# broadinstitute/Tangram

Measured on NVIDIA H100. Metric: map_cells_to_space iterations/sec, higher is better.
Workload: dtype bf16 operands / f32 accumulate+state

## Files before the change

### tangram_b200/csrc/adam_rows.cuh

```cuda
#pragma once
#include "common.cuh"
#include "gemm_tc.cuh"

namespace tgb {

struct AdamRowsArgs {
  float* M; __nv_bfloat16* m; float* v;
  const __nv_bfloat16* dq;
  __nv_bfloat16* Pt;
  const RowConst* rowc;
  float* zsum; float* pxsum; float* l1sum; float* l2sum;
  int ld, V, row0, row1;
  float lam_r, lam_l1, lam_l2;
  AdamScalars a;
};

__device__ __forceinline__ void ldg256f(const float* src, float (&x)[8]) {
  asm volatile("ld.global.cs.v4.f32 {%0,%1,%2,%3}, [%8];\n\t"
               "ld.global.cs.v4.f32 {%4,%5,%6,%7}, [%8+16];"
               : "=f"(x[0]), "=f"(x[1]), "=f"(x[2]), "=f"(x[3]), "=f"(x[4]), "=f"(x[5]), "=f"(x[6]), "=f"(x[7]) : "l"(src));
}
__device__ __forceinline__ void stg256f(float* dst, const float (&x)[8]) {
  asm volatile("st.global.cs.v4.f32 [%0], {%1,%2,%3,%4};\n\t"
               "st.global.cs.v4.f32 [%0+16], {%5,%6,%7,%8};"
// ... 13 lines not shown
  for (int e = 0; e < 4; ++e) {
    const __nv_bfloat162 b = *reinterpret_cast<const __nv_bfloat162*>(&w[e]);
    f[2 * e] = __low2float(b); f[2 * e + 1] = __high2float(b);
  }
}
__device__ __forceinline__ uint4 pack_bf8(const float (&f)[8]) {
  uint4 o;
  __nv_bfloat162 b;
  b = __floats2bfloat162_rn(f[0], f[1]); o.x = *reinterpret_cast<uint32_t*>(&b);
  b = __floats2bfloat162_rn(f[2], f[3]); o.y = *reinterpret_cast<uint32_t*>(&b);
  b = __floats2bfloat162_rn(f[4], f[5]); o.z = *reinterpret_cast<uint32_t*>(&b);
  b = __floats2bfloat162_rn(f[6], f[7]); o.w = *reinterpret_cast<uint32_t*>(&b);
  return o;
}

#ifndef TGB_ADAM_MAXNREG
#define TGB_ADAM_MAXNREG 96
#endif
template <bool PLAIN>
__global__ void __maxnreg__(TGB_ADAM_MAXNREG)
k_adam_rows(const AdamRowsArgs p) {
  const int lane = threadIdx.x & 31;
  const int row = p.row0 + blockIdx.x * 8 + (threadIdx.x >> 5);
  if (row >= p.row1) return;
  const RowConst rc = p.rowc[row];
  const float lse_l2e = rc.lse * 1.4426950408889634f;
  const size_t base = (size_t)row * p.ld;
  float* Mr = p.M + base; __nv_bfloat16* mr = p.m + base; float* vr = p.v + base;
  const __nv_bfloat16* dr = p.dq + base;
  __nv_bfloat16* pr = p.Pt + base;

  const float k_nstep = -p.a.step_size;

  float zs = 0.f, pxs = 0.f, l1s = 0.f, l2s = 0.f;

  auto load = [&](int c, AdamRowsLoad& L) {
    ldg256f(Mr + c, L.x); L.mq = ldg128_stream(mr + c); ldg256f(vr + c, L.v);
    L.d = ldg128_stream(dr + c);
  };
// ... 70 lines not shown
  if (c < p.ld) {
    AdamRowsLoad A;
    load(c, A);
    process(c, A);
  }
  zs = warp_sum(zs);
  if (p.pxsum) pxs = warp_sum(pxs);
  if (p.l1sum) { l1s = warp_sum(l1s); l2s = warp_sum(l2s); }
  if (lane == 0) {
    p.zsum[row] = zs;
    if (p.pxsum) p.pxsum[row] = pxs;
    if (p.l1sum) { p.l1sum[row] = l1s; p.l2sum[row] = l2s; }
  }
}

struct AdamRowsExactArgs {
  float* M; float* m; float* v;
  const float* dp;
  const RowStat* stats; const float* rdot;
  int ld, V, row0, row1;
  float lam_r, lam_l1, lam_l2;
  AdamScalars a;
};

__global__ void __launch_bounds__(256)
k_adam_rows_exact(const AdamRowsExactArgs p) {
  const int lane = threadIdx.x & 31;
  const int row = p.row0 + blockIdx.x * 8 + (threadIdx.x >> 5);
  if (row >= p.row1) return;
  const RowStat st = p.stats[row];
// ... 15 lines not shown
        if (p.lam_l2 != 0.f) g += 2.f * p.lam_l2 * x[e];
        x[e] = adam_update(x[e], g, m[e], v[e], p.a);
      }
    }
    stg256f(Mr + c, x); stg256f(mr + c, m); stg256f(vr + c, v);
  }
}

static inline int adam_rows_exact_launch(const AdamRowsExactArgs& a, cudaStream_t s) {
  const int rows = a.row1 - a.row0;
  if (rows <= 0) return 0;
  k_adam_rows_exact<<<(unsigned)ceil_div(rows, 8), 256, 0, s>>>(a);
  return cudaGetLastError() == cudaSuccess ? 0 : -2;
}

static inline int adam_rows_launch(const AdamRowsArgs& a, cudaStream_t s) {
  const int rows = a.row1 - a.row0;
  if (rows <= 0) return 0;
  const unsigned grid = (unsigned)ceil_div(rows, 8);
  const bool plain = a.lam_r == 0.f && a.lam_l1 == 0.f && a.lam_l2 == 0.f;
  if (plain) k_adam_rows<true><<<grid, 256, 0, s>>>(a);
  else k_adam_rows<false><<<grid, 256, 0, s>>>(a);
  return cudaGetLastError() == cudaSuccess ? 0 : -2;
}

}
```

### tangram_b200/csrc/gemm_tc.cuh

```cuda
#pragma once
#include <cuda.h>
#include <cstdio>
#include "common.cuh"
#include "gemm_simt.cuh"

namespace tgb {

constexpr int TC_BM = 128;
constexpr int TC_BK = 64;
constexpr int TC_MMA_K = 16;
constexpr int TC_BN = 256;
constexpr int TC_THREADS = 384;
constexpr int TC_ACC = TC_BN / 2;

__device__ __forceinline__ uint32_t smem_u32(const void* p) { return (uint32_t)__cvta_generic_to_shared(p); }

__device__ __forceinline__ void mbar_init(uint64_t* bar, uint32_t count) {
  asm volatile("mbarrier.init.shared::cta.b64 [%0], %1;" ::"r"(smem_u32(bar)), "r"(count));
}
__device__ __forceinline__ void mbar_expect_tx(uint64_t* bar, uint32_t bytes) {
  asm volatile("mbarrier.arrive.expect_tx.shared::cta.b64 _, [%0], %1;" ::"r"(smem_u32(bar)), "r"(bytes) : "memory");
}
__device__ __forceinline__ void mbar_wait(uint64_t* bar, uint32_t parity) {
  asm volatile(
// ... 486 lines not shown
  const long long kps = ((k_total + s - 1) / s + TC_BK - 1) / TC_BK * TC_BK;
  return (int)((k_total + kps - 1) / kps);
}
static inline int tc_splits_for_chain(long long k_total, int max_chain) {
  long long s = (k_total + max_chain - 1) / max_chain;
  if (s < 1) s = 1;
  const long long kps = ((k_total + s - 1) / s + TC_BK - 1) / TC_BK * TC_BK;
  return (int)((k_total + kps - 1) / kps);
}
static inline int tc_forward_splits(int num_sms, int N, int V, int Ke) {
  return tc_splits(num_sms, (long long)ceil_div(V, TC_BM) * ceil_div(Ke, TC_BN), N, 512);
}
static inline int tc_kps(int k_total, int splits) {
  return (int)(round_up(ceil_div(k_total, splits), TC_BK));
}
static inline unsigned tc_grid(const TcContext& tc, long long total) {
  return (unsigned)(total < tc.num_sms ? total : tc.num_sms);
}

static inline int tc_make_maps(TcContext& tc, TcMaps* maps, const __nv_bfloat16* base, size_t plane_elems, int n_planes,
                               uint64_t cols, uint64_t rows, uint64_t ld, uint32_t bi, uint32_t bo, char* err, size_t n) {
  for (int p = 0; p < 3; ++p) {
    const __nv_bfloat16* ptr = base + (size_t)(p < n_planes ? p : 0) * plane_elems;
    if (tc_make_map(tc, &maps->m[p], ptr, cols, rows, ld, bi, bo, err, n)) return -2;
  }
  return 0;
}

struct TcPlan {
  TcMaps a, b;
  CUtensorMap pt, dq;
  bool ready = false;
};

static inline int tc_forward_plan(TcContext& tc, TcPlan& pl, const __nv_bfloat16* P, size_t p_plane, const __nv_bfloat16* Sx,
                                  size_t s_plane, int planes, int N, int V, int Ke, int ld, char* err, size_t n) {
  if (tc_make_maps(tc, &pl.a, P, p_plane, planes, V, N, ld, 64, 64, err, n)) return -2;
  if (tc_make_maps(tc, &pl.b, Sx, s_plane, planes, Ke, N, Ke, 64, 64, err, n)) return -2;
  pl.ready = true;
  return 0;
}
static inline int tc_forward_launch(TcContext& tc, const TcPlan& pl, int n_pairs, float* out, int N, int V, int Ke, int splits,
                                    cudaStream_t s, char* err, size_t n) {
  auto kern = k_gemm_tc<false, false, tc_stages<TcEpiStore>(), TcEpiStore>;
  if (tc_set_smem(tc, kern, TC_SMEM, err, n)) return -2;
  TcEpiStore epi{out, Ke, (size_t)V * Ke, V, 0};
  const int tm = (int)ceil_div(V, TC_BM), tn = (int)ceil_div(Ke, TC_BN);
  kern<<<tc_grid(tc, (long long)tm * tn * splits), TC_THREADS, TC_SMEM, s>>>(pl.a, pl.b, n_pairs, N, tc_kps(N, splits), tm, tn,
                                                                             splits, 1, kPolicyEvictNormal, kPolicyEvictNormal, 0, 0, epi);
  return tc_check_launch("tc_gemm_fwd", err, n);
}
static inline int tc_forward_launch_rows(TcContext& tc, const TcPlan& pl, float* out, int accumulate, int row0, int row1, int V, int Ke,
                                         cudaStream_t s, char* err, size_t n) {
  auto kern = k_gemm_tc<false, false, tc_stages<TcEpiStore>(), TcEpiStore>;
  if (tc_set_smem(tc, kern, TC_SMEM, err, n)) return -2;
  TcEpiStore epi{out, Ke, (size_t)V * Ke, V, accumulate};
  const int tm = (int)ceil_div(V, TC_BM), tn = (int)ceil_div(Ke, TC_BN);
  kern<<<tc_grid(tc, (long long)tm * tn), TC_THREADS, TC_SMEM, s>>>(pl.a, pl.b, 1, row1, (int)round_up(row1 - row0, TC_BK), tm, tn,
                                                                    1, 1, kPolicyEvictNormal, kPolicyEvictNormal, 0, row0, epi);
  return tc_check_launch("tc_gemm_fwd", err, n);
}
static inline int tc_forward(TcContext& tc, const __nv_bfloat16* P, size_t p_plane, const __nv_bfloat16* Sx, size_t s_plane,
                             int n_pairs, float* out, int N, int V, int Ke, int ld, int splits, cudaStream_t s, char* err,
                             size_t n) {
  TcPlan pl;
  if (tc_forward_plan(tc, pl, P, p_plane, Sx, s_plane, n_pairs > 1 ? 3 : 1, N, V, Ke, ld, err, n)) return -2;
  return tc_forward_launch(tc, pl, n_pairs, out, N, V, Ke, splits, s, err, n);
}

static inline int tc_dpstore_plan(TcContext& tc, TcPlan& pl, const __nv_bfloat16* Sxb, size_t s_plane, const __nv_bfloat16* dYb,
                                  size_t dy_plane, int planes, int N, int V, int Ke, char* err, size_t n) {
  if (tc_make_maps(tc, &pl.a, Sxb, s_plane, planes, Ke, N, Ke, 64, TC_BM, err, n)) return -2;
  if (tc_make_maps(tc, &pl.b, dYb, dy_plane, planes, Ke, V, Ke, 64, TC_BN, err, n)) return -2;
  pl.ready = true;
  return 0;
}
static inline int tc_dpstore_epi_plan(TcContext& tc, TcPlan& pl, const __nv_bfloat16* Pt, const __nv_bfloat16* dq, int N, int ld,
                                      char* err, size_t n) {
  if (tc_make_map(tc, &pl.pt, Pt, ld, N, ld, 64, 64, err, n)) return -2;
  return tc_make_map(tc, &pl.dq, dq, ld, N, ld, 64, 64, err, n);
}
template <class Epi>
static inline int tc_dpstore_launch(TcContext& tc, const TcPlan& pl, int n_pairs, const Epi& epi, int row0, int row1, int V, int Ke,
                                    cudaStream_t s, char* err, size_t n) {
  const int tn = (int)ceil_div(V, TC_BN);
  auto kern = k_gemm_tc<true, true, tc_stages<Epi>(), Epi>;
  constexpr int smem = tc_smem<Epi>();
  if (tc_set_smem(tc, kern, smem, err, n)) return -2;
  const int tm0 = row0 / TC_BM, tm = (int)ceil_div(row1, TC_BM) - tm0;
  kern<<<tc_grid(tc, (long long)tm * tn), TC_THREADS, smem, s>>>(pl.a, pl.b, n_pairs, Ke, Ke, tm, tn, 1, 1,
                                                                 kPolicyEvictNormal, kPolicyEvictLast, tm0, 0, epi);
  return tc_check_launch("tc_gemm_bwd_dp", err, n);
}

}
```

### tangram_b200/csrc/tangram_b200.cu

```cuda
#include "../../include/tangram_b200.h"

#include <algorithm>
#include <cmath>
#include <cstdarg>
#include <cstdio>
#include <cstdlib>
#include <cstring>
#include <mutex>
#include <string>
#include <thread>
#include <vector>

#include "common.cuh"
#include "kernels_elem.cuh"
#include "gemm_simt.cuh"
#include "gemm_tc.cuh"
#include "adam_rows.cuh"
#include "legacy_rng.cuh"
#include "agreement.cuh"
#include "annotate.cuh"
#include "mt19937_jump.h"
#include "nccl_dl.h"

using namespace tgb;
// ... 98 lines not shown
  DevBuf<float> colfin;
  DevBuf<float> hist;
  int64_t hist_len = 0, hist_cap = 0;
  bool have_expr = false, have_density = false, have_ct = false, have_mapping = false;
  bool in_step = false;
  int64_t launches = 0;
  float legacy_stats[8] = {0};
  TcContext tc;
  TcPlan plan_fwd, plan_dp;
  DevBuf<__nv_bfloat16> dq;
  DevBuf<__nv_bfloat16> mb;
  DevBuf<float> rcenter;
  DevBuf<float> dpf;
  bool pipelined = false;
  int nchunks = 1, chunk_row[9] = {0};
  cudaStream_t hi = nullptr, lo = nullptr, sf = nullptr;
  cudaEvent_t ev_fork = nullptr, ev_join_hi = nullptr, ev_join_lo = nullptr, ev_join_sf = nullptr, ev_loss = nullptr;
  cudaEvent_t ev_g[8] = {}, ev_a[8] = {}, ev_f[8] = {};
  bool a_valid = false;
  bool prefetch_next = false;
  bool fwd_ahead = false;
  bool defer_join = false;
  bool serial = false;
  bool recording = false;
  std::vector<LaunchRecord> records;
  void drop_records(size_t from) {
    for (size_t i = from; i < records.size(); ++i) cudaEventDestroy(records[i].ev);
    records.resize(from);
  }
  void* comm = nullptr;
  bool comm_owned = false;
  int comm_rank = 0, comm_world = 1;
  bool y_nccl = false;
  void* y_reg = nullptr;
  void release_exchange_registration() {
    if (!y_nccl) return;
    char e[64];
    if (NcclApi* a = nccl_api(e, sizeof(e))) {
      if (y_reg && comm) a->CommDeregister(comm, y_reg);
      a->MemFree(Y.p);
    }
    Y.p = nullptr; Y.n = 0; y_nccl = false; y_reg = nullptr;
  }
  ~tgb200_mapper() {
    release_exchange_registration();
    if (comm && comm_owned) { char e[64]; if (NcclApi* a = nccl_api(e, sizeof(e))) a->CommDestroy(comm); }
    if (hi) cudaStreamDestroy(hi);
    if (lo) cudaStreamDestroy(lo);
    if (sf) cudaStreamDestroy(sf);
    for (cudaEvent_t e : {ev_fork, ev_join_hi, ev_join_lo, ev_join_sf, ev_loss}) if (e) cudaEventDestroy(e);
    for (int i = 0; i < 8; ++i)
      for (cudaEvent_t e : {ev_g[i], ev_a[i], ev_f[i]}) if (e) cudaEventDestroy(e);
    drop_records(0);
  }
};

static void mark(tgb200_mapper* h, cudaStream_t s, const char* name) {
  h->launches++;
  if (!h->recording) return;
  cudaEvent_t e;
  cudaEventCreate(&e);
  cudaEventRecord(e, s);
  h->records.push_back({name, s == h->hi ? 1 : (s == h->lo ? 2 : (s == h->sf ? 3 : 0)), e});
}
#define LAUNCH_CHECK(name)                                                                  \
  do {                                                                                      \
    cudaError_t e__ = cudaGetLastError();                                                   \
    if (e__ != cudaSuccess) return fail(TGB200_ERR_CUDA, "launch %s: %s", name, cudaGetErrorString(e__)); \
    mark(h, s, name);                                                                       \
  } while (0)

static float* s_act(tgb200_mapper* h) { return h->constrained ? h->Sf.p : h->Sx.p; }

static bool needs_rowaux(const tgb200_config& c) { return c.lambda_l1 != 0.f || c.lambda_l2 != 0.f; }
static bool needs_rowscalars(const tgb200_config& c) {
  return c.lambda_r != 0.f || c.lambda_l1 != 0.f || c.lambda_l2 != 0.f;
}

extern "C" int tgb200_host_pin(void* buf, int64_t bytes, int32_t threads, int32_t device) {
  if (!buf || bytes <= 0) return fail(TGB200_ERR_INVALID, "bad argument");
  CK(cudaSetDevice(device));
  const size_t page = 4096, n = (size_t)bytes;
  const int nt = threads < 1 ? 1 : (threads > 32 ? 32 : threads);
  volatile unsigned char* b = static_cast<volatile unsigned char*>(buf);
  auto touch = [=](size_t lo, size_t hi) { for (size_t o = lo; o < hi; o += page) b[o] = 0; };
// ... 85 lines not shown
  A(h->d.alloc(h->V)); A(h->dsrc.alloc(h->N));
  A(h->stats.alloc(h->N)); A(h->rowaux.alloc((size_t)2 * h->N)); A(h->rdot.alloc(h->N));
  if (h->bf16) {
    int nc = h->N >= 32768 ? 4 : (h->N >= 8192 ? 2 : 1);
    if (const char* e = getenv("TGB200_CHUNKS")) nc = atoi(e);
    if (nc < 1) nc = 1;
    if (nc > 8) nc = 8;
    if (h->constrained) nc = 1;
    while (nc > 1 && h->N / nc < 1024) --nc;
    h->nchunks = nc;
    for (int c = 0; c <= nc; ++c) h->chunk_row[c] = c == nc ? h->N : (int)round_up((int64_t)c * h->N / nc, 256);
  }
  if (h->nchunks > 1) {
    int lo_p = 0, hi_p = 0;
    cudaDeviceGetStreamPriorityRange(&lo_p, &hi_p);
    const int mid_p = hi_p < lo_p ? hi_p + 1 : lo_p;
    bool ok = cudaStreamCreateWithPriority(&h->hi, cudaStreamNonBlocking, hi_p) == cudaSuccess &&
              cudaStreamCreateWithPriority(&h->sf, cudaStreamNonBlocking, mid_p) == cudaSuccess &&
              cudaStreamCreateWithPriority(&h->lo, cudaStreamNonBlocking, lo_p) == cudaSuccess;
    cudaEvent_t* evs[5] = {&h->ev_fork, &h->ev_join_hi, &h->ev_join_lo, &h->ev_join_sf, &h->ev_loss};
    for (auto e : evs) ok = ok && cudaEventCreateWithFlags(e, cudaEventDisableTiming) == cudaSuccess;
    for (int c = 0; c < 8; ++c)
      ok = ok && cudaEventCreateWithFlags(&h->ev_g[c], cudaEventDisableTiming) == cudaSuccess &&
           cudaEventCreateWithFlags(&h->ev_a[c], cudaEventDisableTiming) == cudaSuccess &&
           cudaEventCreateWithFlags(&h->ev_f[c], cudaEventDisableTiming) == cudaSuccess;
    if (!ok) A(fail(TGB200_ERR_CUDA, "stream / event creation failed: %s", cudaGetErrorString(cudaGetLastError())));
    h->pipelined = ok;
  }
  h->tc.num_sms = prop.multiProcessorCount;
  if (h->nchunks > 1) {
    h->fwd_splits = 1;
  } else if (h->tcm) {
    h->fwd_splits = tc_forward_splits(h->tc.num_sms, h->N, h->V, h->Ke);
    if (h->x3) h->fwd_splits = std::max(h->fwd_splits, tc_splits_for_chain(h->N, 2048));
  } else {
    const int tiles = (int)(ceil_div(h->V, 128) * ceil_div(h->Ke, 128));
    h->fwd_splits = std::clamp((int)ceil_div(2 * h->tc.num_sms, tiles), 1, (int)ceil_div(h->N, 512));
  }
  if (h->fwd_splits > 1) A(h->Ypart.alloc((size_t)h->fwd_splits * vk));
  A(h->Y.alloc(vk + kTail));
  if (!h->tcm) A(h->dY.alloc(vk));
  if (h->constrained) {
    A(h->Fl.alloc(h->N)); A(h->mF.alloc(h->N)); A(h->vF.alloc(h->N)); A(h->fsig.alloc(h->N));
    A(h->Sf.alloc((size_t)h->N * h->Ke)); A(h->fscal.alloc(4));
// ... 183 lines not shown

static int zero_moments(tgb200_mapper* h, cudaStream_t s) {
  if (h->bf16) CK(cudaMemsetAsync(h->mb.p, 0, h->mb.n * sizeof(__nv_bfloat16), s));
  else CK(cudaMemsetAsync(h->m.p, 0, h->m.n * sizeof(float), s));
  CK(cudaMemsetAsync(h->v.p, 0, h->v.n * sizeof(float), s));
  return TGB200_OK;
}

static int reset_optimizer(tgb200_mapper* h, cudaStream_t s) {
  CKS(zero_moments(h, s));
  if (h->bf16) CK(cudaMemsetAsync(h->rcenter.p, 0, h->rcenter.n * sizeof(float), s));
  h->step = 0;
  h->hist_len = 0;
  h->in_step = false;
  h->p_state = PState::stale;
  h->fwd_ahead = false;
  return TGB200_OK;
}

extern "C" int tgb200_reset_adam(tgb200_mapper* h, void* stream) {
  if (!h) return fail(TGB200_ERR_INVALID, "null handle");
  if (h->in_step) return fail(TGB200_ERR_STATE, "reset_adam inside a step");
  cudaStream_t s = (cudaStream_t)stream;
  CK(cudaSetDevice(h->cfg.device));
  CKS(zero_moments(h, s));
  if (h->constrained) {
    CK(cudaMemsetAsync(h->mF.p, 0, h->mF.n * sizeof(float), s));
    CK(cudaMemsetAsync(h->vF.p, 0, h->vF.n * sizeof(float), s));
  }
  h->step = 0;
  return TGB200_OK;
// ... 339 lines not shown

static cudaStream_t work_stream(tgb200_mapper* h, cudaStream_t s) { return (h->pipelined && !h->serial) ? h->hi : s; }
static cudaStream_t update_stream(tgb200_mapper* h, cudaStream_t s) { return (h->pipelined && !h->serial) ? h->lo : s; }
static int fork_streams(tgb200_mapper* h, cudaStream_t s) {
  if (!h->pipelined || h->serial || h->defer_join) return TGB200_OK;
  CK(cudaEventRecord(h->ev_fork, s));
  CK(cudaStreamWaitEvent(h->hi, h->ev_fork, 0));
  return TGB200_OK;
}
static int join_streams(tgb200_mapper* h, cudaStream_t s) {
  if (!h->pipelined || h->serial || h->defer_join) return TGB200_OK;
  CK(cudaEventRecord(h->ev_join_hi, h->hi));
  CK(cudaStreamWaitEvent(s, h->ev_join_hi, 0));
  CK(cudaEventRecord(h->ev_join_lo, h->lo));
  CK(cudaStreamWaitEvent(s, h->ev_join_lo, 0));
  CK(cudaEventRecord(h->ev_join_sf, h->sf));
  CK(cudaStreamWaitEvent(s, h->ev_join_sf, 0));
  return TGB200_OK;
}

static int forward_chunk(tgb200_mapper* h, cudaStream_t s, int c, int fresh, const float* lseA, float* lseT) {
  float* rowaux = needs_rowaux(h->cfg) ? h->rowaux.p : nullptr;
  if (!h->plan_fwd.ready)
    CKS(tc_forward_plan(h->tc, h->plan_fwd, h->Pb.p, (size_t)h->N * h->ld, h->Sxs.p, (size_t)h->N * h->Ke, 1, h->N, h->V, h->Ke, h->ld,
                        g_err, sizeof(g_err)));
  const int r0 = h->nchunks > 1 ? h->chunk_row[c] : 0, r1 = h->nchunks > 1 ? h->chunk_row[c + 1] : h->N;
  if (h->a_valid && h->pipelined && !h->serial) CK(cudaStreamWaitEvent(s, h->ev_a[c], 0));
  k_row_norm<<<(unsigned)ceil_div(r1 - r0, 256), 256, 0, s>>>(fresh, h->zsum.p, h->pxsum.p, h->l1sum.p, h->l2sum.p,
                                                             lseA, lseT, h->inv_zt.p, h->stats.p, rowaux, r0, r1);
  LAUNCH_CHECK("row_norm");
  const long long nq = (long long)(r1 - r0) * (h->Ke / 4);
  k_scale_rows_bf16<<<(unsigned)ceil_div(nq, 256), 256, 0, s>>>(s_act(h), h->inv_zt.p, r0, r1, h->Ke, h->Sxs.p);
  LAUNCH_CHECK("scale_rows");
  if (h->nchunks > 1) {
    CKS(tc_forward_launch_rows(h->tc, h->plan_fwd, h->Y.p, c > 0 ? 1 : 0, r0, r1, h->V, h->Ke, s, g_err, sizeof(g_err)));
    mark(h, s, "tc_gemm_fwd");
  }
  return TGB200_OK;
}

static int forward_pass(tgb200_mapper* h, cudaStream_t s, int want_entropy) {
  float* rowaux = needs_rowaux(h->cfg) ? h->rowaux.p : nullptr;
  if (h->bf16) {
    if (h->p_state == PState::stale) {
      CKS(launch_softmax_rows<__nv_bfloat16>(h, s, h->Pb.p, 1, rowaux));
      h->p_state = PState::fresh;
    }
    if (h->fwd_ahead) {
      h->fwd_ahead = false;
      for (int c = 0; c < h->nchunks; ++c) CK(cudaStreamWaitEvent(s, h->ev_f[c], 0));
      if (h->nchunks > 1) return TGB200_OK;
    } else {
      for (int c = 0; c < h->nchunks; ++c) CKS(forward_chunk(h, s, c, h->p_state == PState::fresh ? 1 : 0, h->lseA, h->lseT));
    }
    if (h->nchunks > 1) return TGB200_OK;
  } else if (h->x3) {
    CKS(launch_softmax_rows<float>(h, s, (float*)nullptr, want_entropy, rowaux, Split3{h->Pb.p, (size_t)h->N * h->ld}));
  } else {
    CKS(launch_softmax_rows<float>(h, s, h->Pf.p, want_entropy, rowaux));
  }
  const size_t vk = (size_t)h->V * h->Ke;
  float* out = h->fwd_splits > 1 ? h->Ypart.p : h->Y.p;
  if (h->tcm) {
    if (!h->plan_fwd.ready) {
      const __nv_bfloat16* sB = h->bf16 ? h->Sxs.p : h->Sxb.p;
      CKS(tc_forward_plan(h->tc, h->plan_fwd, h->Pb.p, (size_t)h->N * h->ld, sB, (size_t)h->N * h->Ke, h->x3 ? 3 : 1, h->N, h->V, h->Ke,
                          h->ld, g_err, sizeof(g_err)));
    }
    CKS(tc_forward_launch(h->tc, h->plan_fwd, h->x3 ? 6 : 1, out, h->N, h->V, h->Ke, h->fwd_splits, s, g_err, sizeof(g_err)));
// ... 124 lines not shown

static int filter_update(tgb200_mapper* h, cudaStream_t s, const AdamScalars& a) {
  const AdamScalarsF af{a.one_minus_beta1, a.beta2, a.one_minus_beta2, a.step_size, a.bc2_sqrt, a.eps};
  k_filter_update<<<(unsigned)ceil_div(h->N, 256), 256, 0, s>>>(h->N, h->rdot.p, h->fsig.p, h->fscal.p, h->cfg.lambda_count,
                                                                 h->cfg.lambda_f_reg, af, h->Fl.p, h->mF.p, h->vF.p);
  LAUNCH_CHECK("filter_update");
  return TGB200_OK;
}

static int backward_bf16(tgb200_mapper* h, cudaStream_t s, cudaStream_t su, const AdamScalars& a) {
  if (!h->plan_dp.ready) {
    CKS(tc_dpstore_epi_plan(h->tc, h->plan_dp, h->Pb.p, h->dq.p, h->N, h->ld, g_err, sizeof(g_err)));
    CKS(tc_dpstore_plan(h->tc, h->plan_dp, h->Sxb.p, 0, h->dYb.p, 0, 1, h->N, h->V, h->Ke, g_err, sizeof(g_err)));
  }
  const bool two_streams = su != s;
  const bool prefetch = two_streams && h->prefetch_next && h->nchunks > 1 && !h->constrained;
  for (int c = 0; c < h->nchunks; ++c) {
    const int r0 = h->nchunks > 1 ? h->chunk_row[c] : 0, r1 = h->nchunks > 1 ? h->chunk_row[c + 1] : h->N;
    TcEpiDpStore epi{h->plan_dp.pt, h->plan_dp.dq, h->ld, h->rcenter.p, h->rpart.p, h->N};
    CKS(tc_dpstore_launch(h->tc, h->plan_dp, 1, epi, r0, r1, h->V, h->Ke, s, g_err, sizeof(g_err)));
    mark(h, s, "tc_gemm_bwd_dp");
    if (two_streams) {
      CK(cudaEventRecord(h->ev_g[c], s));
      CK(cudaStreamWaitEvent(su, h->ev_g[c], 0));
    }
    k_rowdot_finalize_staged<<<(unsigned)ceil_div(r1 - r0, 256), 256, 0, su>>>(h->rpart.p, h->r_parts, h->N, r0, r1, h->lseT, h->inv_zt.p,
                                                                               h->stats.p, h->rcenter.p, h->rdot.p, h->rowc.p);
    { cudaStream_t s = su; LAUNCH_CHECK("rowdot_finalize"); }
    if (h->constrained) CKS(filter_update(h, su, a));
    AdamRowsArgs ar{h->M.p, h->mb.p, h->v.p, h->dq.p, h->Pb.p, reinterpret_cast<const RowConst*>(h->rowc.p),
                    h->zsum.p, h->pxsum.p, h->l1sum.p, h->l2sum.p, h->ld, h->V, r0, r1,
                    h->cfg.lambda_r, h->cfg.lambda_l1, h->cfg.lambda_l2, a};
    if (adam_rows_launch(ar, su)) return fail(TGB200_ERR_CUDA, "launch adam_rows: %s", cudaGetErrorString(cudaGetLastError()));
    mark(h, su, "adam_rows");
    if (two_streams) CK(cudaEventRecord(h->ev_a[c], su));
    h->a_valid = two_streams;
    if (prefetch) {
      if (c == 0) CK(cudaStreamWaitEvent(h->sf, h->ev_loss, 0));
      CKS(forward_chunk(h, h->sf, c, 0, h->lseT, h->lseA));
      CK(cudaEventRecord(h->ev_f[c], h->sf));
    }
  }
  h->fwd_ahead = prefetch;
  float* t = h->lseA; h->lseA = h->lseT; h->lseT = t;
  h->p_state = PState::updated;
  return TGB200_OK;
}

static int backward_bf16x3(tgb200_mapper* h, cudaStream_t s, const AdamScalars& a) {
  const size_t nkp = (size_t)h->N * h->Ke, vkp = (size_t)h->V * h->Ke, nvp = (size_t)h->N * h->ld;
  if (!h->plan_dp.ready)
    CKS(tc_dpstore_plan(h->tc, h->plan_dp, h->Sxb.p, nkp, h->dYb.p, vkp, 3, h->N, h->V, h->Ke, g_err, sizeof(g_err)));
  TcEpiDpStoreF32 epi{h->dpf.p, h->ld, h->Pb.p, nvp, h->rpart.p, h->N};
  CKS(tc_dpstore_launch(h->tc, h->plan_dp, 6, epi, 0, h->N, h->V, h->Ke, s, g_err, sizeof(g_err)));
  mark(h, s, "tc_gemm_bwd_dp");
  k_rowdot_finalize<<<(unsigned)ceil_div(h->N, 256), 256, 0, s>>>(h->rpart.p, h->r_parts, h->N, h->rdot.p);
  LAUNCH_CHECK("rowdot_finalize");
  if (h->constrained) CKS(filter_update(h, s, a));
  AdamRowsExactArgs ar{h->M.p, h->m.p, h->v.p, h->dpf.p, h->stats.p, h->rdot.p, h->ld, h->V, 0, h->N,
                       h->cfg.lambda_r, h->cfg.lambda_l1, h->cfg.lambda_l2, a};
  if (adam_rows_exact_launch(ar, s)) return fail(TGB200_ERR_CUDA, "launch adam_rows_exact: %s", cudaGetErrorString(cudaGetLastError()));
  mark(h, s, "adam_rows");
  return TGB200_OK;
}

static int backward_fp32(tgb200_mapper* h, cudaStream_t s, const AdamScalars& a) {
  GemmArgs g;
  g.A = h->Pf.p; g.lda = h->ld; g.B = h->dY.p; g.ldb = h->Ke;
  g.M = h->N; g.N = h->Ke; g.K = h->V; g.k_per_split = (int)round_up(h->V, 16);
// ... 12 lines not shown
  LAUNCH_CHECK("simt_gemm_bwd_adam");
  return TGB200_OK;
}

extern "C" int tgb200_step_end(tgb200_mapper* h, float lr, void* stream) {
  if (!h) return fail(TGB200_ERR_INVALID, "null handle");
  cudaStream_t caller = (cudaStream_t)stream;
  CK(cudaSetDevice(h->cfg.device));
  if (!h->in_step) return fail(TGB200_ERR_STATE, "step_end without step_begin");
  CKS(ensure_history(h, h->hist_len + 1, caller));
  CKS(fork_streams(h, caller));
  cudaStream_t s = work_stream(h, caller);
  float* hist_row = h->hist.p + (size_t)h->hist_len * TGB200_HIST_COLS;
  const bool sharded = h->cfg.n_cells_global != h->N;
  CKS(loss_stage(h, s, hist_row, !sharded));
  if (h->pipelined && !h->serial) CK(cudaEventRecord(h->ev_loss, s));

  const AdamScalars a = adam_scalars(h->cfg, h->step + 1, lr);
  if (h->bf16) CKS(backward_bf16(h, s, update_stream(h, caller), a));
  else if (h->x3) CKS(backward_bf16x3(h, s, a));
  else CKS(backward_fp32(h, s, a));
  CKS(join_streams(h, caller));
  h->step++;
  h->hist_len++;
  h->in_step = false;
  return TGB200_OK;
}

static int exchange_partials(tgb200_mapper* h, cudaStream_t s) {
  NcclApi* api = nccl_api(g_err, sizeof(g_err));
  if (!api) return TGB200_ERR_STATE;
// ... 85 lines not shown

extern "C" int tgb200_run(tgb200_mapper* h, int32_t n_steps, float lr, void* stream) {
  if (!h) return fail(TGB200_ERR_INVALID, "null handle");
  if (n_steps < 0) return fail(TGB200_ERR_INVALID, "n_steps < 0");
  const bool sharded = h->cfg.n_cells_global != h->N;
  if (sharded && !h->comm)
    return fail(TGB200_ERR_STATE, "cell-sharded handle without a communicator: call tgb200_comm_init_rank / tgb200_set_comm, or drive "
                                  "step_begin / all-reduce / step_end yourself");
  CK(cudaSetDevice(h->cfg.device));
  CKS(ensure_history(h, h->hist_len + n_steps, (cudaStream_t)stream));
  if (n_steps == 0) return TGB200_OK;
  CKS(fork_streams(h, (cudaStream_t)stream));
  h->defer_join = true;
  int st = TGB200_OK;
  for (int i = 0; i < n_steps && st == TGB200_OK; ++i) {
    h->prefetch_next = i + 1 < n_steps;
    st = tgb200_step_begin(h, stream);
    if (st == TGB200_OK && sharded) st = exchange_partials(h, work_stream(h, (cudaStream_t)stream));
    if (st == TGB200_OK) st = tgb200_step_end(h, lr, stream);
  }
  h->defer_join = false;
  h->prefetch_next = false;
  CKS(join_streams(h, (cudaStream_t)stream));
  return st;
}

extern "C" int tgb200_history_len(tgb200_mapper* h, int64_t* n) {
  if (!h || !n) return fail(TGB200_ERR_INVALID, "null argument");
  *n = h->hist_len;
  return TGB200_OK;
}

extern "C" int tgb200_get_history(tgb200_mapper* h, int64_t first, int64_t count, float* out, void* stream) {
  if (!h || (!out && count > 0)) return fail(TGB200_ERR_INVALID, "null argument");
  if (first < 0 || count < 0 || first + count > h->hist_len) return fail(TGB200_ERR_INVALID, "history range [%lld,%lld) outside [0,%lld)", (long long)first, (long long)(first + count), (long long)h->hist_len);
  if (count == 0) return TGB200_OK;
  cudaStream_t s = (cudaStream_t)stream;
// ... 56 lines not shown
  }
  if (v) CK(cudaMemcpy2DAsync(v, w, h->v.p, pitch, w, h->N, cudaMemcpyDefault, s));
  if (step) *step = h->step;
  CK(cudaStreamSynchronize(s));
  return TGB200_OK;
}

extern "C" int tgb200_set_state(tgb200_mapper* h, const float* M, const float* m, const float* v, int64_t step, void* stream) {
  if (!h) return fail(TGB200_ERR_INVALID, "null handle");
  if (step < 0) return fail(TGB200_ERR_INVALID, "step < 0");
  cudaStream_t s = (cudaStream_t)stream;
  CK(cudaSetDevice(h->cfg.device));
  const size_t w = (size_t)h->V * sizeof(float), pitch = (size_t)h->ld * sizeof(float);
  if (M) {
    CK(cudaMemcpy2DAsync(h->M.p, pitch, M, w, w, h->N, cudaMemcpyDefault, s)); h->have_mapping = true; h->p_state = PState::stale;
    h->fwd_ahead = false;
    if (h->bf16) CK(cudaMemsetAsync(h->rcenter.p, 0, h->rcenter.n * sizeof(float), s));
  }
  if (m && !h->bf16) CK(cudaMemcpy2DAsync(h->m.p, pitch, m, w, w, h->N, cudaMemcpyDefault, s));
  if (m && h->bf16) {
    float* scratch;
    int blk;
    DevBuf<float> one_row;
    CKS(moment_scratch(h, one_row, &scratch, &blk));
    for (int r0 = 0; r0 < h->N; r0 += blk) {
      const int nr = h->N - r0 < blk ? h->N - r0 : blk;
      const long long n = (long long)nr * h->ld;
      CK(cudaMemsetAsync(scratch, 0, (size_t)n * sizeof(float), s));
      CK(cudaMemcpy2DAsync(scratch, pitch, m + (size_t)r0 * h->V, w, w, nr, cudaMemcpyDefault, s));
      k_f32_to_bf16<<<(unsigned)ceil_div(n, 256), 256, 0, s>>>(scratch, h->mb.p + (size_t)r0 * h->ld, n);
      LAUNCH_CHECK("f32_to_bf16");
// ... 62 lines not shown
    LAUNCH_CHECK("simt_gemm_project");
    CK(cudaMemcpy2DAsync(out + c0, (size_t)n_cols * sizeof(float), Oc.p, (size_t)ldc * sizeof(float),
                         (size_t)nc * sizeof(float), h->V, cudaMemcpyDefault, s));
  }
  CK(cudaStreamSynchronize(s));
  return TGB200_OK;
}

extern "C" int tgb200_validation_terms(tgb200_mapper* h, float* out4, void* stream) {
  if (!h || !out4) return fail(TGB200_ERR_INVALID, "null argument");
  cudaStream_t s = (cudaStream_t)stream;
  CK(cudaSetDevice(h->cfg.device));
  CKS(check_ready(h));
  if (h->in_step) return fail(TGB200_ERR_STATE, "validation_terms inside a step");
  if (h->cfg.n_cells_global != h->N) return fail(TGB200_ERR_UNSUPPORTED, "validation_terms on a sharded handle");
  if (h->bf16) { h->p_state = PState::stale; h->fwd_ahead = false; }
  CKS(forward_pass(h, s, 1));
  LossParams p = make_loss_params(h);
  DevBuf<float> rowpart, coefAr, coefBr, hist;
  CKS(rowpart.alloc((size_t)h->ncolchunk * h->V * 2)); CKS(coefAr.alloc(h->V)); CKS(coefBr.alloc(h->V));
  CKS(hist.alloc(TGB200_HIST_COLS));
  p.rowpart = rowpart.p; p.coefAr = coefAr.p; p.coefBr = coefBr.p;
  p.lam_g2 = 1.f; p.lam_g1 = 1.f; p.lam_nb = 0.f; p.lam_go = 0.f; p.lam_ct = 0.f; p.density_mode = 0;
  CKS(reduce_columns(h, s, p, true, 1));
  k_row_scalar_reduce<<<1, 1024, 0, s>>>(h->stats.p, nullptr, nullptr, h->N, h->Y.p + (size_t)h->V * h->Ke);
  LAUNCH_CHECK("row_scalar_reduce");
  k_loss_scalars<<<1, 1024, 0, s>>>(p, 1, h->nredchunk, hist.p);
  LAUNCH_CHECK("loss_scalars");
  std::vector<float> hrow(TGB200_HIST_COLS), cA(h->K), cB(h->K), Gh((size_t)h->V * h->Ke), tail(4);
  CK(cudaMemcpyAsync(hrow.data(), hist.p, sizeof(float) * TGB200_HIST_COLS, cudaMemcpyDeviceToHost, s));
  CK(cudaMemcpyAsync(cA.data(), h->coefA.p, sizeof(float) * h->K, cudaMemcpyDeviceToHost, s));
// ... 328 lines not shown
```

Baseline: 43.83.

## Partition SMs between persistent Adam update and concurrent GEMMs, drop forward prefetch stream

Replaces the one-warp-per-row Adam launch with a persistent grid capped at a fixed SM budget (512-thread blocks looping over rows), and shrinks the grid of the backward dp GEMM and the next forward GEMM by the same number of SMs so the update kernel on the low-priority stream can run beside them without contending for SMs. The separate forward-prefetch stream and its events are removed, so the next step's forward chunks now run on the main stream, sized to leave room for any pending update. This trades speculative cross-step overlap for explicit spatial SM partitioning. The risks are that the GEMMs lose SMs and the update kernel may become bandwidth-starved on only about 32 SMs.

```diff
diff --git a/tangram_b200/csrc/adam_rows.cuh b/tangram_b200/csrc/adam_rows.cuh
--- a/tangram_b200/csrc/adam_rows.cuh
+++ b/tangram_b200/csrc/adam_rows.cuh
@@ -51,15 +51,8 @@
   return o;
 }
 
-#ifndef TGB_ADAM_MAXNREG
-#define TGB_ADAM_MAXNREG 96
-#endif
 template <bool PLAIN>
-__global__ void __maxnreg__(TGB_ADAM_MAXNREG)
-k_adam_rows(const AdamRowsArgs p) {
-  const int lane = threadIdx.x & 31;
-  const int row = p.row0 + blockIdx.x * 8 + (threadIdx.x >> 5);
-  if (row >= p.row1) return;
+__device__ __forceinline__ void adam_row(const AdamRowsArgs& p, int row, int lane) {
   const RowConst rc = p.rowc[row];
   const float lse_l2e = rc.lse * 1.4426950408889634f;
   const size_t base = (size_t)row * p.ld;
@@ -160,6 +153,19 @@
   }
 }
 
+constexpr int ADAM_THREADS = 512;
+constexpr int ADAM_WARPS = ADAM_THREADS / 32;
+#ifndef TGB_ADAM_MAXNREG
+#define TGB_ADAM_MAXNREG 96
+#endif
+template <bool PLAIN>
+__global__ void __maxnreg__(TGB_ADAM_MAXNREG)
+k_adam_rows(const AdamRowsArgs p) {
+  const int lane = threadIdx.x & 31;
+  for (int row = p.row0 + blockIdx.x * ADAM_WARPS + (threadIdx.x >> 5); row < p.row1; row += gridDim.x * ADAM_WARPS)
+    adam_row<PLAIN>(p, row, lane);
+}
+
 struct AdamRowsExactArgs {
   float* M; float* m; float* v;
   const float* dp;
@@ -205,13 +211,14 @@
   return cudaGetLastError() == cudaSuccess ? 0 : -2;
 }
 
-static inline int adam_rows_launch(const AdamRowsArgs& a, cudaStream_t s) {
+static inline int adam_rows_launch(const AdamRowsArgs& a, int sms, cudaStream_t s) {
   const int rows = a.row1 - a.row0;
   if (rows <= 0) return 0;
-  const unsigned grid = (unsigned)ceil_div(rows, 8);
+  const long long need = ceil_div(rows, ADAM_WARPS);
+  const unsigned grid = (unsigned)(need < sms ? need : sms);
   const bool plain = a.lam_r == 0.f && a.lam_l1 == 0.f && a.lam_l2 == 0.f;
-  if (plain) k_adam_rows<true><<<grid, 256, 0, s>>>(a);
-  else k_adam_rows<false><<<grid, 256, 0, s>>>(a);
+  if (plain) k_adam_rows<true><<<grid, ADAM_THREADS, 0, s>>>(a);
+  else k_adam_rows<false><<<grid, ADAM_THREADS, 0, s>>>(a);
   return cudaGetLastError() == cudaSuccess ? 0 : -2;
 }
 
diff --git a/tangram_b200/csrc/gemm_tc.cuh b/tangram_b200/csrc/gemm_tc.cuh
--- a/tangram_b200/csrc/gemm_tc.cuh
+++ b/tangram_b200/csrc/gemm_tc.cuh
@@ -524,8 +524,8 @@
 static inline int tc_kps(int k_total, int splits) {
   return (int)(round_up(ceil_div(k_total, splits), TC_BK));
 }
-static inline unsigned tc_grid(const TcContext& tc, long long total) {
-  return (unsigned)(total < tc.num_sms ? total : tc.num_sms);
+static inline unsigned tc_grid(int sms, long long total) {
+  return (unsigned)(total < sms ? total : sms);
 }
 
 static inline int tc_make_maps(TcContext& tc, TcMaps* maps, const __nv_bfloat16* base, size_t plane_elems, int n_planes,
@@ -556,17 +556,17 @@
   if (tc_set_smem(tc, kern, TC_SMEM, err, n)) return -2;
   TcEpiStore epi{out, Ke, (size_t)V * Ke, V, 0};
   const int tm = (int)ceil_div(V, TC_BM), tn = (int)ceil_div(Ke, TC_BN);
-  kern<<<tc_grid(tc, (long long)tm * tn * splits), TC_THREADS, TC_SMEM, s>>>(pl.a, pl.b, n_pairs, N, tc_kps(N, splits), tm, tn,
+  kern<<<tc_grid(tc.num_sms, (long long)tm * tn * splits), TC_THREADS, TC_SMEM, s>>>(pl.a, pl.b, n_pairs, N, tc_kps(N, splits), tm, tn,
                                                                              splits, 1, kPolicyEvictNormal, kPolicyEvictNormal, 0, 0, epi);
   return tc_check_launch("tc_gemm_fwd", err, n);
 }
 static inline int tc_forward_launch_rows(TcContext& tc, const TcPlan& pl, float* out, int accumulate, int row0, int row1, int V, int Ke,
-                                         cudaStream_t s, char* err, size_t n) {
+                                         int sms, cudaStream_t s, char* err, size_t n) {
   auto kern = k_gemm_tc<false, false, tc_stages<TcEpiStore>(), TcEpiStore>;
   if (tc_set_smem(tc, kern, TC_SMEM, err, n)) return -2;
   TcEpiStore epi{out, Ke, (size_t)V * Ke, V, accumulate};
   const int tm = (int)ceil_div(V, TC_BM), tn = (int)ceil_div(Ke, TC_BN);
-  kern<<<tc_grid(tc, (long long)tm * tn), TC_THREADS, TC_SMEM, s>>>(pl.a, pl.b, 1, row1, (int)round_up(row1 - row0, TC_BK), tm, tn,
+  kern<<<tc_grid(sms, (long long)tm * tn), TC_THREADS, TC_SMEM, s>>>(pl.a, pl.b, 1, row1, (int)round_up(row1 - row0, TC_BK), tm, tn,
                                                                     1, 1, kPolicyEvictNormal, kPolicyEvictNormal, 0, row0, epi);
   return tc_check_launch("tc_gemm_fwd", err, n);
 }
@@ -592,13 +592,13 @@
 }
 template <class Epi>
 static inline int tc_dpstore_launch(TcContext& tc, const TcPlan& pl, int n_pairs, const Epi& epi, int row0, int row1, int V, int Ke,
-                                    cudaStream_t s, char* err, size_t n) {
+                                    int sms, cudaStream_t s, char* err, size_t n) {
   const int tn = (int)ceil_div(V, TC_BN);
   auto kern = k_gemm_tc<true, true, tc_stages<Epi>(), Epi>;
   constexpr int smem = tc_smem<Epi>();
   if (tc_set_smem(tc, kern, smem, err, n)) return -2;
   const int tm0 = row0 / TC_BM, tm = (int)ceil_div(row1, TC_BM) - tm0;
-  kern<<<tc_grid(tc, (long long)tm * tn), TC_THREADS, smem, s>>>(pl.a, pl.b, n_pairs, Ke, Ke, tm, tn, 1, 1,
+  kern<<<tc_grid(sms, (long long)tm * tn), TC_THREADS, smem, s>>>(pl.a, pl.b, n_pairs, Ke, Ke, tm, tn, 1, 1,
                                                                  kPolicyEvictNormal, kPolicyEvictLast, tm0, 0, epi);
   return tc_check_launch("tc_gemm_bwd_dp", err, n);
 }
diff --git a/tangram_b200/csrc/tangram_b200.cu b/tangram_b200/csrc/tangram_b200.cu
--- a/tangram_b200/csrc/tangram_b200.cu
+++ b/tangram_b200/csrc/tangram_b200.cu
@@ -136,12 +136,12 @@
   DevBuf<float> dpf;
   bool pipelined = false;
   int nchunks = 1, chunk_row[9] = {0};
-  cudaStream_t hi = nullptr, lo = nullptr, sf = nullptr;
-  cudaEvent_t ev_fork = nullptr, ev_join_hi = nullptr, ev_join_lo = nullptr, ev_join_sf = nullptr, ev_loss = nullptr;
-  cudaEvent_t ev_g[8] = {}, ev_a[8] = {}, ev_f[8] = {};
+  int update_sms = 0;
+  cudaStream_t hi = nullptr, lo = nullptr;
+  cudaEvent_t ev_fork = nullptr, ev_join_hi = nullptr, ev_join_lo = nullptr;
+  cudaEvent_t ev_g[8] = {}, ev_a[8] = {};
   bool a_valid = false;
-  bool prefetch_next = false;
-  bool fwd_ahead = false;
+  bool update_pending = false;
   bool defer_join = false;
   bool serial = false;
   bool recording = false;
@@ -169,10 +169,9 @@
     if (comm && comm_owned) { char e[64]; if (NcclApi* a = nccl_api(e, sizeof(e))) a->CommDestroy(comm); }
     if (hi) cudaStreamDestroy(hi);
     if (lo) cudaStreamDestroy(lo);
-    if (sf) cudaStreamDestroy(sf);
-    for (cudaEvent_t e : {ev_fork, ev_join_hi, ev_join_lo, ev_join_sf, ev_loss}) if (e) cudaEventDestroy(e);
+    for (cudaEvent_t e : {ev_fork, ev_join_hi, ev_join_lo}) if (e) cudaEventDestroy(e);
     for (int i = 0; i < 8; ++i)
-      for (cudaEvent_t e : {ev_g[i], ev_a[i], ev_f[i]}) if (e) cudaEventDestroy(e);
+      for (cudaEvent_t e : {ev_g[i], ev_a[i]}) if (e) cudaEventDestroy(e);
     drop_records(0);
   }
 };
@@ -183,7 +182,7 @@
   cudaEvent_t e;
   cudaEventCreate(&e);
   cudaEventRecord(e, s);
-  h->records.push_back({name, s == h->hi ? 1 : (s == h->lo ? 2 : (s == h->sf ? 3 : 0)), e});
+  h->records.push_back({name, s == h->hi ? 1 : (s == h->lo ? 2 : 0), e});
 }
 #define LAUNCH_CHECK(name)                                                                  \
   do {                                                                                      \
@@ -191,6 +190,11 @@
     if (e__ != cudaSuccess) return fail(TGB200_ERR_CUDA, "launch %s: %s", name, cudaGetErrorString(e__)); \
     mark(h, s, name);                                                                       \
   } while (0)
+
+#ifndef TGB_UPDATE_SMS
+#define TGB_UPDATE_SMS 32
+#endif
+static int update_sms_for(int num_sms) { return std::clamp((num_sms * TGB_UPDATE_SMS + 66) / 132, 1, num_sms - 1); }
 
 static float* s_act(tgb200_mapper* h) { return h->constrained ? h->Sf.p : h->Sx.p; }
 
@@ -306,20 +310,18 @@
   if (h->nchunks > 1) {
     int lo_p = 0, hi_p = 0;
     cudaDeviceGetStreamPriorityRange(&lo_p, &hi_p);
-    const int mid_p = hi_p < lo_p ? hi_p + 1 : lo_p;
     bool ok = cudaStreamCreateWithPriority(&h->hi, cudaStreamNonBlocking, hi_p) == cudaSuccess &&
-              cudaStreamCreateWithPriority(&h->sf, cudaStreamNonBlocking, mid_p) == cudaSuccess &&
               cudaStreamCreateWithPriority(&h->lo, cudaStreamNonBlocking, lo_p) == cudaSuccess;
-    cudaEvent_t* evs[5] = {&h->ev_fork, &h->ev_join_hi, &h->ev_join_lo, &h->ev_join_sf, &h->ev_loss};
+    cudaEvent_t* evs[3] = {&h->ev_fork, &h->ev_join_hi, &h->ev_join_lo};
     for (auto e : evs) ok = ok && cudaEventCreateWithFlags(e, cudaEventDisableTiming) == cudaSuccess;
     for (int c = 0; c < 8; ++c)
       ok = ok && cudaEventCreateWithFlags(&h->ev_g[c], cudaEventDisableTiming) == cudaSuccess &&
-           cudaEventCreateWithFlags(&h->ev_a[c], cudaEventDisableTiming) == cudaSuccess &&
-           cudaEventCreateWithFlags(&h->ev_f[c], cudaEventDisableTiming) == cudaSuccess;
+           cudaEventCreateWithFlags(&h->ev_a[c], cudaEventDisableTiming) == cudaSuccess;
     if (!ok) A(fail(TGB200_ERR_CUDA, "stream / event creation failed: %s", cudaGetErrorString(cudaGetLastError())));
     h->pipelined = ok;
   }
   h->tc.num_sms = prop.multiProcessorCount;
+  h->update_sms = update_sms_for(h->tc.num_sms);
   if (h->nchunks > 1) {
     h->fwd_splits = 1;
   } else if (h->tcm) {
@@ -533,7 +535,6 @@
   h->hist_len = 0;
   h->in_step = false;
   h->p_state = PState::stale;
-  h->fwd_ahead = false;
   return TGB200_OK;
 }
 
@@ -903,8 +904,7 @@
   CK(cudaStreamWaitEvent(s, h->ev_join_hi, 0));
   CK(cudaEventRecord(h->ev_join_lo, h->lo));
   CK(cudaStreamWaitEvent(s, h->ev_join_lo, 0));
-  CK(cudaEventRecord(h->ev_join_sf, h->sf));
-  CK(cudaStreamWaitEvent(s, h->ev_join_sf, 0));
+  h->update_pending = false;
   return TGB200_OK;
 }
 
@@ -922,7 +922,9 @@
   k_scale_rows_bf16<<<(unsigned)ceil_div(nq, 256), 256, 0, s>>>(s_act(h), h->inv_zt.p, r0, r1, h->Ke, h->Sxs.p);
   LAUNCH_CHECK("scale_rows");
   if (h->nchunks > 1) {
-    CKS(tc_forward_launch_rows(h->tc, h->plan_fwd, h->Y.p, c > 0 ? 1 : 0, r0, r1, h->V, h->Ke, s, g_err, sizeof(g_err)));
+    const bool beside = h->update_pending && c + 1 < h->nchunks;
+    CKS(tc_forward_launch_rows(h->tc, h->plan_fwd, h->Y.p, c > 0 ? 1 : 0, r0, r1, h->V, h->Ke,
+                               beside ? h->tc.num_sms - h->update_sms : h->tc.num_sms, s, g_err, sizeof(g_err)));
     mark(h, s, "tc_gemm_fwd");
   }
   return TGB200_OK;
@@ -935,13 +937,7 @@
       CKS(launch_softmax_rows<__nv_bfloat16>(h, s, h->Pb.p, 1, rowaux));
       h->p_state = PState::fresh;
     }
-    if (h->fwd_ahead) {
-      h->fwd_ahead = false;
-      for (int c = 0; c < h->nchunks; ++c) CK(cudaStreamWaitEvent(s, h->ev_f[c], 0));
-      if (h->nchunks > 1) return TGB200_OK;
-    } else {
-      for (int c = 0; c < h->nchunks; ++c) CKS(forward_chunk(h, s, c, h->p_state == PState::fresh ? 1 : 0, h->lseA, h->lseT));
-    }
+    for (int c = 0; c < h->nchunks; ++c) CKS(forward_chunk(h, s, c, h->p_state == PState::fresh ? 1 : 0, h->lseA, h->lseT));
     if (h->nchunks > 1) return TGB200_OK;
   } else if (h->x3) {
     CKS(launch_softmax_rows<float>(h, s, (float*)nullptr, want_entropy, rowaux, Split3{h->Pb.p, (size_t)h->N * h->ld}));
@@ -1096,11 +1092,17 @@
     CKS(tc_dpstore_plan(h->tc, h->plan_dp, h->Sxb.p, 0, h->dYb.p, 0, 1, h->N, h->V, h->Ke, g_err, sizeof(g_err)));
   }
   const bool two_streams = su != s;
-  const bool prefetch = two_streams && h->prefetch_next && h->nchunks > 1 && !h->constrained;
+  const int num_sms = h->tc.num_sms;
+#ifdef TGB_SERIAL_UPDATE_ON_K
+  const int upd_sms = h->update_sms;
+#else
+  const int upd_sms = two_streams ? h->update_sms : num_sms;
+#endif
   for (int c = 0; c < h->nchunks; ++c) {
     const int r0 = h->nchunks > 1 ? h->chunk_row[c] : 0, r1 = h->nchunks > 1 ? h->chunk_row[c + 1] : h->N;
     TcEpiDpStore epi{h->plan_dp.pt, h->plan_dp.dq, h->ld, h->rcenter.p, h->rpart.p, h->N};
-    CKS(tc_dpstore_launch(h->tc, h->plan_dp, 1, epi, r0, r1, h->V, h->Ke, s, g_err, sizeof(g_err)));
+    CKS(tc_dpstore_launch(h->tc, h->plan_dp, 1, epi, r0, r1, h->V, h->Ke, two_streams && c > 0 ? num_sms - h->update_sms : num_sms, s,
+                          g_err, sizeof(g_err)));
     mark(h, s, "tc_gemm_bwd_dp");
     if (two_streams) {
       CK(cudaEventRecord(h->ev_g[c], s));
@@ -1113,17 +1115,13 @@
     AdamRowsArgs ar{h->M.p, h->mb.p, h->v.p, h->dq.p, h->Pb.p, reinterpret_cast<const RowConst*>(h->rowc.p),
                     h->zsum.p, h->pxsum.p, h->l1sum.p, h->l2sum.p, h->ld, h->V, r0, r1,
                     h->cfg.lambda_r, h->cfg.lambda_l1, h->cfg.lambda_l2, a};
-    if (adam_rows_launch(ar, su)) return fail(TGB200_ERR_CUDA, "launch adam_rows: %s", cudaGetErrorString(cudaGetLastError()));
+    if (adam_rows_launch(ar, upd_sms, su))
+      return fail(TGB200_ERR_CUDA, "launch adam_rows: %s", cudaGetErrorString(cudaGetLastError()));
     mark(h, su, "adam_rows");
     if (two_streams) CK(cudaEventRecord(h->ev_a[c], su));
     h->a_valid = two_streams;
-    if (prefetch) {
-      if (c == 0) CK(cudaStreamWaitEvent(h->sf, h->ev_loss, 0));
-      CKS(forward_chunk(h, h->sf, c, 0, h->lseT, h->lseA));
-      CK(cudaEventRecord(h->ev_f[c], h->sf));
-    }
-  }
-  h->fwd_ahead = prefetch;
+    h->update_pending = two_streams;
+  }
   float* t = h->lseA; h->lseA = h->lseT; h->lseT = t;
   h->p_state = PState::updated;
   return TGB200_OK;
@@ -1134,7 +1132,7 @@
   if (!h->plan_dp.ready)
     CKS(tc_dpstore_plan(h->tc, h->plan_dp, h->Sxb.p, nkp, h->dYb.p, vkp, 3, h->N, h->V, h->Ke, g_err, sizeof(g_err)));
   TcEpiDpStoreF32 epi{h->dpf.p, h->ld, h->Pb.p, nvp, h->rpart.p, h->N};
-  CKS(tc_dpstore_launch(h->tc, h->plan_dp, 6, epi, 0, h->N, h->V, h->Ke, s, g_err, sizeof(g_err)));
+  CKS(tc_dpstore_launch(h->tc, h->plan_dp, 6, epi, 0, h->N, h->V, h->Ke, h->tc.num_sms, s, g_err, sizeof(g_err)));
   mark(h, s, "tc_gemm_bwd_dp");
   k_rowdot_finalize<<<(unsigned)ceil_div(h->N, 256), 256, 0, s>>>(h->rpart.p, h->r_parts, h->N, h->rdot.p);
   LAUNCH_CHECK("rowdot_finalize");
@@ -1177,7 +1175,6 @@
   float* hist_row = h->hist.p + (size_t)h->hist_len * TGB200_HIST_COLS;
   const bool sharded = h->cfg.n_cells_global != h->N;
   CKS(loss_stage(h, s, hist_row, !sharded));
-  if (h->pipelined && !h->serial) CK(cudaEventRecord(h->ev_loss, s));
 
   const AdamScalars a = adam_scalars(h->cfg, h->step + 1, lr);
   if (h->bf16) CKS(backward_bf16(h, s, update_stream(h, caller), a));
@@ -1293,13 +1290,11 @@
   h->defer_join = true;
   int st = TGB200_OK;
   for (int i = 0; i < n_steps && st == TGB200_OK; ++i) {
-    h->prefetch_next = i + 1 < n_steps;
     st = tgb200_step_begin(h, stream);
     if (st == TGB200_OK && sharded) st = exchange_partials(h, work_stream(h, (cudaStream_t)stream));
     if (st == TGB200_OK) st = tgb200_step_end(h, lr, stream);
   }
   h->defer_join = false;
-  h->prefetch_next = false;
   CKS(join_streams(h, (cudaStream_t)stream));
   return st;
 }
@@ -1386,7 +1381,6 @@
   const size_t w = (size_t)h->V * sizeof(float), pitch = (size_t)h->ld * sizeof(float);
   if (M) {
     CK(cudaMemcpy2DAsync(h->M.p, pitch, M, w, w, h->N, cudaMemcpyDefault, s)); h->have_mapping = true; h->p_state = PState::stale;
-    h->fwd_ahead = false;
     if (h->bf16) CK(cudaMemsetAsync(h->rcenter.p, 0, h->rcenter.n * sizeof(float), s));
   }
   if (m && !h->bf16) CK(cudaMemcpy2DAsync(h->m.p, pitch, m, w, w, h->N, cudaMemcpyDefault, s));
@@ -1479,7 +1473,7 @@
   CKS(check_ready(h));
   if (h->in_step) return fail(TGB200_ERR_STATE, "validation_terms inside a step");
   if (h->cfg.n_cells_global != h->N) return fail(TGB200_ERR_UNSUPPORTED, "validation_terms on a sharded handle");
-  if (h->bf16) { h->p_state = PState::stale; h->fwd_ahead = false; }
+  if (h->bf16) h->p_state = PState::stale;
   CKS(forward_pass(h, s, 1));
   LossParams p = make_loss_params(h);
   DevBuf<float> rowpart, coefAr, coefBr, hist;
```

New measurement: 47.94, median of 6. 1.09x the previous value.
